# TopHillRobotics/quadruped-robot

Measured on AMD Instinct MI355X. Metric: MPC+WBC control ticks/s (batched robots), higher is better.
Workload: dtype f32 assembly / f64 QP+WBC

## Files before the change

### quadruped-robot_amd/csrc/qr_wbc_kernel.hip

```cpp
#include <hip/hip_runtime.h>
#include <type_traits>
#include "qr_device_types.h"
#include "qr_wave_helpers.h"
#include "qr_kernels.h"
#include "qr_wbc_rigid_body.h"

namespace qrgpu {

#ifdef QR_TIMELINE
#define QW_P_TL pipe.tl
#define QW_P_TLR pipe.tlr
#else
#define QW_P_TL ((long long *)nullptr)
#define QW_P_TLR ((int *)nullptr)
#endif

__device__ __forceinline__ real wsum(real v) { return wave_sum_d(v); }

__device__ __forceinline__ real dot18(const real *a, int as, const real *b, int bs, int k)
{
    real av[18], bv[18];
#pragma unroll
    for (int t = 0; t < 18; ++t) { const bool ok = t < k; av[t] = ok ? a[t * as] : 0.0; bv[t] = ok ? b[t * bs] : 0.0; }
    real s0 = 0.0, s1 = 0.0, s2 = 0.0;
#pragma unroll
    for (int t = 0; t < 18; t += 3) { s0 += av[t] * bv[t]; s1 += av[t + 1] * bv[t + 1]; s2 += av[t + 2] * bv[t + 2]; }
    return (s0 + s1) + s2;
}

__device__ __forceinline__ int fdiv16(int e, int rcp) { return (e * rcp) >> 16; }
__device__ __forceinline__ int rcp16(int n) { return (65536 + n - 1) / n; }

template <int KMAX>
__device__ __forceinline__ void gemm(int lane, real *C, int ldc, const real *A, int lda, bool tA, const real *B, int ldb, bool tB,
                                     int m, int n, int k, real alpha = 1.0, real beta = 0.0, const real *C0 = nullptr, int ldc0 = 0)
{
    const int rn = rcp16(n);
    const int as = tA ? lda : 1, bs = tB ? 1 : ldb;
    for (int e = lane; e < m * n; e += 64) {
        const int i = fdiv16(e, rn), j = e - i * n;
        const real *ap = tA ? A + i : A + i * lda;
        const real *bp = tB ? B + j * ldb : B + j;
        real av[KMAX], bv[KMAX];
#pragma unroll
        for (int t = 0; t < KMAX; ++t) { const bool ok = t < k; av[t] = ok ? ap[t * as] : 0.0; bv[t] = ok ? bp[t * bs] : 0.0; }
        real a0 = 0.0, a1 = 0.0, a2 = 0.0;
#pragma unroll
        for (int t = 0; t < KMAX; t += 3) {
            a0 += av[t] * bv[t];
            if (t + 1 < KMAX) a1 += av[t + 1] * bv[t + 1];
            if (t + 2 < KMAX) a2 += av[t + 2] * bv[t + 2];
        }
        real v = alpha * ((a0 + a1) + a2);
        if (C0) v += beta * C0[i * ldc0 + j];
        C[i * ldc + j] = v;
    }
    wave_sync();
}

template <int UMAX>
__device__ __forceinline__ real spd_inverse(int lane, real *A, int ld, int n, real *col)
{
    const int rn = rcp16(n);
    int ei[UMAX], ej[UMAX];
    real a[UMAX];
#pragma unroll
    for (int u = 0; u < UMAX; ++u) {
        const int e = lane + 64 * u;
        const bool ok = e < n * n;
        ei[u] = ok ? fdiv16(e, rn) : -1;
        ej[u] = ok ? e - ei[u] * n : -1;
        a[u] = ok ? A[ei[u] * ld + ej[u]] : 0.0;
    }
    real minpiv = 1e300;
    for (int k = 0; k < n; ++k) {
#pragma unroll
        for (int u = 0; u < UMAX; ++u) if (ej[u] == k) col[ei[u]] = a[u];
        wave_sync();
        const real piv = col[k];
        minpiv = piv < minpiv ? piv : minpiv;
        const real ip = fast_rcp(piv);
        real ci[UMAX], cj[UMAX];
#pragma unroll
        for (int u = 0; u < UMAX; ++u) { const bool ok = ei[u] >= 0; ci[u] = ok ? col[ei[u]] : 0.0; cj[u] = ok ? col[ej[u]] : 0.0; }
#pragma unroll
        for (int u = 0; u < UMAX; ++u) {
            if (ei[u] == k) a[u] = (ej[u] == k) ? -ip : cj[u] * ip;
            else if (ej[u] == k) a[u] = ci[u] * ip;
            else a[u] -= ci[u] * cj[u] * ip;
        }
        wave_sync();
    }
#pragma unroll
    for (int u = 0; u < UMAX; ++u) if (ei[u] >= 0) A[ei[u] * ld + ej[u]] = -a[u];
    wave_sync();
    return minpiv;
}

template <int UMAX = 3>
__device__ __forceinline__ void psd_pinv(int lane, const real *W, int n, real thr, real *Winv, real *scr)
{
    if (n == 1) {
        if (lane == 0) Winv[0] = (W[0] > thr) ? 1.0 / W[0] : 0.0;
        wave_sync();
        return;
    }
    for (int e = lane; e < n * n; e += 64) Winv[e] = W[e];
    wave_sync();
    const real minpiv = spd_inverse<UMAX>(lane, Winv, n, n, scr);
    real fro = 0.0;
    for (int e = lane; e < n * n; e += 64) fro += Winv[e] * Winv[e];
    fro = wsum(fro);
    const bool full_rank = (minpiv > 0.0) && (fro == fro) && (1.0 > thr * __builtin_sqrt(fro));
    if (full_rank) return;
    if (lane == 0) {
        real *Am = scr;
        real *V = Winv;
        for (int i = 0; i < n; ++i)
            for (int j = 0; j < n; ++j) { Am[i * n + j] = 0.5 * (W[i * n + j] + W[j * n + i]); V[i * n + j] = (i == j) ? 1.0 : 0.0; }
        for (int sweep = 0; sweep < 30; ++sweep) {
            real off = 0.0;
            for (int p = 0; p < n; ++p) for (int q2 = p + 1; q2 < n; ++q2) off += Am[p * n + q2] * Am[p * n + q2];
            if (off < 1e-40) break;
            for (int p = 0; p < n - 1; ++p)
                for (int q2 = p + 1; q2 < n; ++q2) {
                    const real apq = Am[p * n + q2];
                    if (apq == 0.0) continue;
                    const real th = (Am[q2 * n + q2] - Am[p * n + p]) / (2.0 * apq);
                    const real t = (th >= 0 ? 1.0 : -1.0) / (fabs(th) + __builtin_sqrt(th * th + 1.0));
                    const real c = 1.0 / __builtin_sqrt(t * t + 1.0), s = t * c;
                    for (int k = 0; k < n; ++k) { const real akp = Am[k * n + p], akq = Am[k * n + q2]; Am[k * n + p] = c * akp - s * akq; Am[k * n + q2] = s * akp + c * akq; }
                    for (int k = 0; k < n; ++k) { const real apk = Am[p * n + k], aqk = Am[q2 * n + k]; Am[p * n + k] = c * apk - s * aqk; Am[q2 * n + k] = s * apk + c * aqk; }
                    for (int k = 0; k < n; ++k) { const real vkp = V[k * n + p], vkq = V[k * n + q2]; V[k * n + p] = c * vkp - s * vkq; V[k * n + q2] = s * vkp + c * vkq; }
                }
        }
        real *ev = scr + n * n;
        for (int i = 0; i < n; ++i) { const real l = fabs(Am[i * n + i]); ev[i] = (l > thr) ? 1.0 / Am[i * n + i] : 0.0; }
        for (int i = 0; i < n; ++i) for (int j = 0; j < n; ++j) Am[i * n + j] = V[i * n + j] * ev[j];
        real *tmp = scr + n * n + n;
        for (int i = 0; i < n; ++i) for (int j = 0; j < n; ++j) { real a = 0; for (int k = 0; k < n; ++k) a += Am[i * n + k] * V[j * n + k]; tmp[i * n + j] = a; }
        for (int e = 0; e < n * n; ++e) Winv[e] = tmp[e];
    }
    wave_sync();
}

__device__ __forceinline__ bool sym3_inverse(const real *W, real thr, real iv[6])
{
    const real a = W[0], b = W[3], c = W[4], d = W[6], e = W[7], f = W[8];
    const real c00 = c * f - e * e, c10 = d * e - b * f, c20 = b * e - c * d, c11 = a * f - d * d, c21 = b * d - a * e, c22 = a * c - b * b;
    const real det = a * c00 + b * c10 + d * c20;
    const real id = 1.0 / det;
    iv[0] = c00 * id; iv[1] = c10 * id; iv[2] = c11 * id; iv[3] = c20 * id; iv[4] = c21 * id; iv[5] = c22 * id;
    const real fro = (iv[0] * iv[0] + iv[2] * iv[2] + iv[5] * iv[5]) + 2.0 * (iv[1] * iv[1] + iv[3] * iv[3] + iv[4] * iv[4]);
    return (a > 0.0) && (c22 > 0.0) && (det > 0.0) && (fro == fro) && (1.0 > thr * __builtin_sqrt(fro));
}

#define QW_NP    0
#define QW_T1    324
#define QW_JB    540
#define QW_JTP   756
#define QW_JTB   810
#define QW_T2    864
#define QW_LAM   918
#define QW_LAMI  1062
#define QW_SCR   1206
#define QW_VEC   1510
#define QW_QP    1564
#define QW_SIZE  1746
#define QR_WBC_SHARED_DOUBLES 1392
#define QR_WBC_LDS_DOUBLES (QR_WBC_SHARED_DOUBLES + 2 * QW_SIZE)

struct QpWork {
    real *tv;
    real *Nq;
    real *Sq;
    real *qd_, *qr_, *qu_, *qc0;
    real *qx;
};
__device__ __forceinline__ QpWork qp_work(real *W)
{
    QpWork q;
    q.tv = W + QW_VEC + 18; q.Nq = W + QW_NP; q.Sq = W + QW_JB;
    q.qd_ = W + QW_QP; q.qr_ = q.qd_ + 32; q.qu_ = q.qr_ + 32; q.qc0 = q.qu_ + 32; q.qx = q.qc0 + 32;
    return q;
}

#define CLEG(k) ((int)((cpack >> (4 * (k))) & 15u))
#define TLEG(k) ((int)((tpack >> (4 * (k))) & 15u))

__device__ __forceinline__ void wbc_signal_done(int *finished, int lane)
{
    if (!finished) return;
    asm volatile("s_waitcnt vmcnt(0)" ::: "memory");
    if (lane == 0) __hip_atomic_fetch_add(finished, 1, __ATOMIC_RELAXED, __HIP_MEMORY_SCOPE_AGENT);
}

__device__ __forceinline__ bool wbc_qp_setup(const int lane, const WbcConst &K, const int nc, const real *A, const real *JC, const real *qdd, const real *Cv, const real *Gv,
                                             real *W, int *sI)
{
    const int dimFr = 3 * nc;
    const QpWork Q = qp_work(W);
    real *tv = Q.tv, *Nq = Q.Nq, *Sq = Q.Sq, *qd_ = Q.qd_, *qx = Q.qx;
    const int nz = 6 + dimFr, np_ = 6, mi = 6 * nc;
    if (lane < 18) {
        real acc = Cv[lane] + Gv[lane];
        for (int k = 0; k < 18; ++k) acc += A[lane * 18 + k] * qdd[k];
        tv[lane] = acc;
    }
    for (int e = lane; e < (np_ + mi) * nz; e += 64) {
        const int c = e / nz, j = e - c * nz;
        real v = 0.0;
        if (c < 6) v = (j < 6) ? A[c * 18 + j] : -JC[(j - 6) * 18 + c];
        else {
            const int u = c - 6, k = u / 6, tt = u - 6 * k;
            if (j >= 6 && (j - 6) / 3 == k) {
                const int ax = (j - 6) - 3 * k;
                if (tt == 0) v = (ax == 2) ? 1.0 : 0.0;
                else if (tt == 5) v = (ax == 2) ? -1.0 : 0.0;
                else { const int a2 = (tt - 1) >> 1; v = (ax == a2) ? (((tt - 1) & 1) ? -1.0 : 1.0) : ((ax == 2) ? (real)K.mu : 0.0); }
            }
        }
        Nq[c * 18 + j] = v;
    }
    if (lane < 18) qx[lane] = 0.0;
    if (lane < 32) sI[32 + lane] = -1;
    wave_sync();
    const real iw_fb = 1.0 / (real)K.w_fb, iw_fr = 1.0 / (real)K.w_fr;
    if (lane < 36) {
        const int a = lane / 6, b2 = lane - 6 * a;
        real acc = 0.0;
        for (int j = 0; j < nz; ++j) acc += Nq[a * 18 + j] * ((j < 6) ? iw_fb : iw_fr) * Nq[b2 * 18 + j];
        Sq[a * 18 + b2] = acc;
    }
    wave_sync();
    real tr = 0.0;
#pragma unroll
    for (int a = 0; a < 6; ++a) tr += Sq[a * 18 + a];
    const real minpiv = spd_inverse<1>(lane, Sq, 18, 6, qd_);
    return !(minpiv > 1e-14 * tr);
}

__device__ __forceinline__ void wbc_qp_and_store(const int lane, const int rid, const int n, const WbcConst &K, const int nc, const unsigned cpack, const bool bad_type,
                                                 const bool eq_dependent, const real *A, const real *JC, const real *cm, real *W, int *sI,
                                                 float *__restrict__ g_tau, int *__restrict__ g_status, const int merge_tau, const int status_or, const int epilogue,
                                                 long long *__restrict__ dbgT, float *__restrict__ g_qp, const bool piped = false, float *__restrict__ g_prev = nullptr)
{
#define QW_TSF(i) do { if (dbgT && (threadIdx.x & 63) == 0 && threadIdx.x < 64) dbgT[(size_t)blockIdx.x * 16 + (i)] = clock64(); } while (0)
    int qp_iters = 0;
    const int dimFr = 3 * nc;
    const QpWork Q = qp_work(W);
    real *tv = Q.tv, *Nq = Q.Nq, *Sq = Q.Sq, *qd_ = Q.qd_, *qr_ = Q.qr_, *qu_ = Q.qu_, *qc0 = Q.qc0, *qx = Q.qx;
    const int nz = 6 + dimFr, np_ = 6, mi = 6 * nc;
    if (lane < 18) {
        real acc = tv[lane];
        for (int k = 0; k < dimFr; ++k) acc -= JC[k * 18 + lane] * cm[51 + 3 * CLEG(k / 3) + k % 3];
        tv[lane] = acc;
    }
    wave_sync();
    if (lane < np_ + mi) {
        const int c = lane;
        real v;
        if (c < 6) v = tv[c];
        else {
            const int u = c - 6, k = u / 6, tt = u - 6 * k;
            real acc = 0.0;
            for (int ax = 0; ax < 3; ++ax) acc += Nq[c * 18 + 6 + 3 * k + ax] * cm[51 + 3 * CLEG(k) + ax];
            v = acc - ((tt == 5) ? -(real)K.max_fz : 0.0);
        }
        qc0[c] = v;
    }
    wave_sync();
    int stw = bad_type ? QRGPU_ST_BAD_TYPE : 0;
    {
        int q = 0;
        const real iw_fb = 1.0 / (real)K.w_fb, iw_fr = 1.0 / (real)K.w_fr;
        auto Minv = [&](int j) -> real { return (j < 6) ? iw_fb : iw_fr; };
        int iter = 0;
        const int maxit = 200;
        int *iter_out = &qp_iters;
        bool fail = false;
        int *act = sI;
        int *posi = sI + 32;
        int next_eq = 0;
        {
            if (eq_dependent) { stw |= QRGPU_ST_WBC_INFEAS; fail = true; }
            if (lane < 6) {
                real acc = 0.0;
#pragma unroll
                for (int b2 = 0; b2 < 6; ++b2) acc -= Sq[lane * 18 + b2] * qc0[b2];
                qu_[lane] = acc; act[lane] = lane; posi[lane] = lane;
            }
            wave_sync();
            if (lane < nz) {
                real acc = 0.0;
#pragma unroll
                for (int a = 0; a < 6; ++a) acc += Nq[a * 18 + lane] * qu_[a];
                qx[lane] = Minv(lane) * acc;
            }
            q = 6; next_eq = np_;
            wave_sync();
        }
        int act_r = (lane < 6) ? lane : 0;
        real u_r = (lane < 6) ? qu_[lane] : 0.0;
        bool active_c = lane < 6;
        const real INF_ = __builtin_inf();
        while (!fail) {
            int p;
            {
                real bs = -1e-10; bool cand = false;
                if (lane >= 6 && lane < np_ + mi && !active_c) {
                    const int cj = 6 + 3 * ((lane - 6) / 6);
                    const real s_ = qc0[lane] + (Nq[lane * 18 + cj] * qx[cj] + Nq[lane * 18 + cj + 1] * qx[cj + 1] + Nq[lane * 18 + cj + 2] * qx[cj + 2]);
                    if (s_ < bs) { bs = s_; cand = true; }
                }
                const real mn = wave_min_d(bs);
                if (!(mn < -1e-10)) break;
                p = first_lane(cand && bs == mn);
                if (p < 0) break;
            }
            real up = 0.0;
            for (;;) {
                if (++iter > maxit) { stw |= QRGPU_ST_WBC_MAXITER; fail = true; break; }
                *iter_out = iter;
                const int pj = 6 + 3 * ((p - 6) / 6);
                const real pn0 = Nq[p * 18 + pj], pn1 = Nq[p * 18 + pj + 1], pn2 = Nq[p * 18 + pj + 2];
                const real delta = (pn0 * pn0 + pn1 * pn1 + pn2 * pn2) * iw_fr;
                const real w0 = iw_fr * pn0, w1 = iw_fr * pn1, w2 = iw_fr * pn2;
                real dq_ = 0.0;
                if (lane < q) { const real *na = Nq + act_r * 18 + pj; dq_ = na[0] * w0 + na[1] * w1 + na[2] * w2; }
                real rq_ = 0.0;
                {
                    const real *Srow = Sq + ((lane < q) ? lane : 0) * 18;
#pragma unroll
                    for (int c = 0; c < 18; c += 6) {
                        if (c >= q) continue;
                        real sv[6];
#pragma unroll
                        for (int j = 0; j < 6; ++j) sv[j] = Srow[c + j];
#pragma unroll
                        for (int j = 0; j < 6; ++j) rq_ += (c + j < q) ? sv[j] * readlane_d(dq_, c + j) : 0.0;
                    }
                    if (lane >= q) rq_ = 0.0;
                }
                const real dr = wave_sum_d(rq_ * dq_);
                const real zc = delta - dr;
                real t1; int lpos;
                {
                    const real tt = (lane < q && act_r >= np_ && rq_ > 0.0) ? u_r * fast_rcp(rq_) : INF_;
                    t1 = wave_min_d(tt);
                    lpos = (t1 < INF_) ? first_lane(tt == t1) : 0x7fffffff;
                }
                const real sp = qc0[p] + (pn0 * qx[pj] + pn1 * qx[pj + 1] + pn2 * qx[pj + 2]);
                const bool have_z = zc > 1e-13 * delta;
                const real izc = fast_rcp(zc);
                const real t2 = have_z ? -sp * izc : INF_;
                const real t = t1 < t2 ? t1 : t2;
                if (!(t < INF_)) { stw |= QRGPU_ST_WBC_INFEAS; fail = true; break; }
                if (have_z) {
                    real acc = 0.0;
                    const int lz = (lane < nz) ? lane : 0;
#pragma unroll
                    for (int c = 0; c < 18; c += 6) {
                        if (c >= q) continue;
                        real nv[6];
#pragma unroll
                        for (int j = 0; j < 6; ++j) nv[j] = Nq[__builtin_amdgcn_readlane(act_r, c + j) * 18 + lz];
#pragma unroll
                        for (int j = 0; j < 6; ++j) acc += (c + j < q) ? nv[j] * readlane_d(rq_, c + j) : 0.0;
                    }
                    if (lane < nz) {
                        const real wl_ = (lane == pj) ? w0 : (lane == pj + 1) ? w1 : (lane == pj + 2) ? w2 : 0.0;
                        qx[lane] += t * (wl_ - Minv(lane) * acc);
                    }
                }
                u_r -= t * rq_;
                up += t;
                if (have_z && t == t2) {
                    const real isg = izc;
                    if (lane < q) qr_[lane] = rq_;
                    wave_sync();
                    { const int rq2 = rcp16(q); for (int e = lane; e < q * q; e += 64) { const int i = fdiv16(e, rq2), j = e - i * q; Sq[i * 18 + j] += qr_[i] * qr_[j] * isg; } }
                    if (lane < q) { Sq[q * 18 + lane] = -rq_ * isg; Sq[lane * 18 + q] = -rq_ * isg; }
                    if (lane == 0) Sq[q * 18 + q] = isg;
                    if (lane == q) { act_r = p; u_r = up; }
                    if (lane == p) active_c = true;
                    ++q;
                    wave_sync();
                    break;
                }
                {
                    const int l = lpos, last = q - 1;
                    const int cdrop = __builtin_amdgcn_readlane(act_r, l), alast = __builtin_amdgcn_readlane(act_r, last);
                    const real ulast = readlane_d(u_r, last);
                    if (lane < q) qd_[lane] = Sq[lane * 18 + l];
                    wave_sync();
                    const real isl = 1.0 / qd_[l];
                    { const int rq2 = rcp16(q); for (int e = lane; e < q * q; e += 64) { const int i = fdiv16(e, rq2), j = e - i * q; if (i != l && j != l) Sq[i * 18 + j] -= qd_[i] * qd_[j] * isl; } }
                    wave_sync();
                    if (l != last) {
                        if (lane < last) qr_[lane] = (lane == l) ? Sq[last * 18 + last] : Sq[last * 18 + lane];
                        wave_sync();
                        if (lane < last) { Sq[l * 18 + lane] = qr_[lane]; Sq[lane * 18 + l] = qr_[lane]; }
                        if (lane == l) { act_r = alast; u_r = ulast; }
                    }
                    if (lane == cdrop) active_c = false;
                    --q;
                    wave_sync();
                }
            }
        }
    }

    QW_TSF(8);
    if (dbgT && threadIdx.x == 0) dbgT[(size_t)blockIdx.x * 16 + 10] = qp_iters;
    if (g_qp) {
        float *o = g_qp + (size_t)rid * 30;
        if (lane < 18) o[lane] = (lane < nz) ? (float)qx[lane] : 0.f;
        if (lane < 12) o[18 + lane] = (lane < dimFr) ? (float)(qx[6 + lane] + cm[51 + 3 * CLEG(lane / 3) + lane % 3]) : 0.f;
    }
    if (lane < 12) {
        const int row = 6 + lane;
        real acc = tv[row];
        for (int k = 0; k < 6; ++k) acc += A[row * 18 + k] * qx[k];
        for (int k = 0; k < dimFr; ++k) acc -= JC[k * 18 + row] * qx[6 + k];
        const int leg = lane / 3;
        const bool stance = cm[63 + leg] != 0.0;
        if (!epilogue) {
            if (!merge_tau || stance) st_through(&g_tau[(size_t)lane * n + rid], (float)acc, piped);
        } else {
            const float t = stance ? (float)acc
                                   : (piped ? __hip_atomic_load(g_tau + (size_t)lane * n + rid, __ATOMIC_RELAXED, __HIP_MEMORY_SCOPE_AGENT) : g_tau[(size_t)lane * n + rid]);
            st_through(&g_tau[(size_t)lane * n + rid], torque_epilogue(t, lane, !stance, epilogue), piped);
        }
    }
    if (g_prev && lane < 3) st_through(&g_prev[(size_t)lane * n + rid], (float)cm[12 + lane], piped);
    if (lane == 0 && g_status) {
        if (status_or & 2) stw |= QRGPU_ST_PIPE_TIMEOUT;
        if (status_or & 1) st_through(&g_status[rid], stw | (piped ? __hip_atomic_load(g_status + rid, __ATOMIC_RELAXED, __HIP_MEMORY_SCOPE_AGENT) : g_status[rid]), piped);
        else st_through(&g_status[rid], stw, piped);
    }
    QW_TSF(9);
#undef QW_TSF
}

#ifdef QR_WBC_DBG_BUILD
#define qr_wbc_kernel qr_wbc_kernel_dbg
#endif
__global__ __launch_bounds__(128, 2)
void qr_wbc_kernel(int n, const WbcConst *__restrict__ types, const int *__restrict__ type_id,
                   const float *__restrict__ g_state, const float *__restrict__ g_cmd, float *__restrict__ g_prev,
                   float *__restrict__ g_tau, float *__restrict__ g_qdes, int *__restrict__ g_status,
                   float *__restrict__ g_dbg, int merge_tau, int status_or, long long *__restrict__ dbgT,
                   const float *__restrict__ g_fr ,
                   int type_ready , int epilogue ,
                   float *__restrict__ g_qp ,
                   WbcPipe pipe )
{
#ifndef QR_WBC_DBG_BUILD
    dbgT = nullptr; g_dbg = nullptr; g_qp = nullptr;
#endif
#define QW_TS(i) do { if (dbgT && threadIdx.x == 0) dbgT[(size_t)blockIdx.x * 16 + (i)] = clock64(); } while (0)
#define QW_TS1(i) do { if (dbgT && threadIdx.x == 64) dbgT[(size_t)blockIdx.x * 16 + (i)] = clock64(); } while (0)
    QW_TS(0);
    int qp_iters = 0;
    int rid = xcd_robot_index((int)blockIdx.x + pipe.slot_base, n);
    const int lane = threadIdx.x & 63;
    const int wv = __builtin_amdgcn_readfirstlane((int)threadIdx.x >> 6);
    const bool gate_gave_up = pipe.gate_abort && __builtin_amdgcn_readfirstlane(*pipe.gate_abort) == (int)pipe.epoch;
    if (pipe.second) {
        if (!gate_gave_up) {
            int cnt = pipe.list_count ? *pipe.list_count : 0;
            cnt = cnt < n ? cnt : n;
            if ((int)blockIdx.x >= cnt) return;
            rid = pipe.list[blockIdx.x];
        }
    }
    if (rid < 0) return;
    if (!pipe.second && gate_gave_up) { wbc_signal_done(pipe.finished, lane); return; }
    if (QW_P_TL && threadIdx.x == 0 && !pipe.second) atomicMin(QW_P_TL + QR_TL_TICKS + (pipe.epoch & 63u) * 8 + 3, wall_clock64());
    if (pipe.order && !pipe.second) rid = pipe.order[rid];
    if (QW_P_TLR && threadIdx.x == 0 && !pipe.second) QW_P_TLR[rid] = (int)wall_clock64();
    int tyid = type_id ? type_id[rid] : 0;
    const bool bad_type = resolve_type(tyid, type_ready);
    const WbcConst &K = types[tyid & (QRGPU_MAX_TYPES - 1)];

    __shared__ real sm[QR_WBC_LDS_DOUBLES];
    real *A = sm;
    real *Ai = A + 324;
    real *JcA = Ai + 324;
    real *JC = JcA + 216;
    real *st = JC + 216;
    real *cm = st + 40;
    real *Gv = cm + 68;
    real *Cv = Gv + 18;
    real *Jcd = Cv + 18;
    real *pGC = Jcd + 12;
    real *vGC = pGC + 12;
    real *tkX = vGC + 12;
    real *tkE = tkX + 18;
    real *tkV = tkE + 18;
    real *legB = tkV + 18;
    real *sRT = legB + 64;
    real *W = sm + QR_WBC_SHARED_DOUBLES + wv * QW_SIZE;
    real *Np = W + QW_NP, *T1 = W + QW_T1, *JB = W + QW_JB, *JtP = W + QW_JTP, *JtB = W + QW_JTB, *T2 = W + QW_T2;
    real *lam = W + QW_LAM, *lamI = W + QW_LAMI, *scr = W + QW_SCR;
    real *qdd = W + QW_VEC, *tv = qdd + 18;
    real *dq1 = qdd, *dq2 = tv;
    __shared__ int sI[64];
    __shared__ int sPipe;
    if (threadIdx.x == 0) sPipe = 0;

    if (wv == 0) {
        if (lane < 37) st[lane] = (real)g_state[(size_t)lane * n + rid];
        for (int e = lane; e < 324; e += 64) A[e] = 0.0;
        for (int e = lane; e < 216; e += 64) JcA[e] = 0.0;
    } else if (g_tau) {
        for (int i = lane; i < 67; i += 64) cm[i] = (real)((g_fr && i >= 51 && i < 63) ? (pipe.flag ? 0.f : g_fr[(size_t)(i - 51) * n + rid]) : g_cmd[(size_t)i * n + rid]);
    }
    __syncthreads();
    const real *quat = st, *pos = st + 4, *bv = st + 7, *qj = st + 13, *qdj = st + 25;
    const xform3 Rwb = quat_to_rot_wb(quat);
    int nc = 0, nt = 2;
    unsigned cpack = 0, tpack = 0;
    if (g_tau) {
#pragma unroll
        for (int l = 0; l < 4; ++l) {
            const int in_contact = __builtin_amdgcn_readfirstlane(cm[63 + l] != 0.0 ? 1 : 0);
            if (in_contact) { cpack |= (unsigned)l << (4 * nc); ++nc; } else { tpack |= (unsigned)l << (4 * (nt - 2)); ++nt; }
        }
    }
    const int dimFr = 3 * nc;

    {
        real *sS = scr + 160, *sC = scr + 176;
        if (lane < 15) {
            const real th = (lane < 12) ? qj[lane] : ((wv == 1 && g_tau) ? cm[9 + lane - 12] : 0.0);
            real s_, c_;
            sincos(th, &s_, &c_);
            sS[lane] = s_; sC[lane] = c_;
        }
        wave_sync();
    }
    const real *sS = scr + 160, *sC = scr + 176;

    QW_TS(1);
    if (wv == 0) {
      if (lane < 4) wbc_leg_inertia_chain(K, Rwb, sS, sC, lane, A, JcA, Gv, legB);
      wave_sync();
      QW_TS(2);
      if (lane == 0) wbc_base_block(K, Rwb, legB, A, Gv);
      wave_sync();
      QW_TS(3);
    } else {
      if (lane < 4) wbc_leg_velocity_chain(K, Rwb, pos, bv, qdj, sS, sC, lane, pGC, vGC, Jcd, Cv, legB);
      wave_sync();
    }
    if (wv == 0) {
    {
        real *Tm = scr, *Um = scr + 72;
        if (lane < 36) {
            const int l = lane / 9, e = lane - 9 * l, i = e / 3, j = e - 3 * i;
            const real *B = A + (6 + 3 * l) * 18 + 6 + 3 * l;
            const real b00 = B[0], b01 = B[1], b02 = B[2], b11 = B[19], b12 = B[20], b22 = B[38];
            const real c00 = b11 * b22 - b12 * b12, c01 = b02 * b12 - b01 * b22, c02 = b01 * b12 - b02 * b11;
            const real c11 = b00 * b22 - b02 * b02, c12 = b01 * b02 - b00 * b12, c22 = b00 * b11 - b01 * b01;
            const real idet = 1.0 / (b00 * c00 + b01 * c01 + b02 * c02);
            const int lo = i < j ? i : j, hi = i < j ? j : i;
            const real c = (lo == 0) ? (hi == 0 ? c00 : (hi == 1 ? c01 : c02)) : (lo == 1 ? (hi == 1 ? c11 : c12) : c22);
            Um[lane] = c * idet;
        }
        wave_sync();
        for (int e = lane; e < 72; e += 64) {
            const int a = e / 12, c = e - 12 * a, l = c / 3, cc = c - 3 * l;
            const real *Ar = A + a * 18 + 6 + 3 * l, *Li = Um + 9 * l;
            Tm[e] = Ar[0] * Li[cc] + Ar[1] * Li[3 + cc] + Ar[2] * Li[6 + cc];
        }
        wave_sync();
        for (int e = lane; e < 144; e += 64) {
            const int c = e / 12, d = e - 12 * c;
            Ai[(6 + c) * 18 + 6 + d] = (c / 3 == d / 3) ? Um[9 * (c / 3) + 3 * (c % 3) + d % 3] : 0.0;
        }
        if (lane < 36) {
            const int a = lane / 6, b2 = lane - 6 * a;
            real acc = A[a * 18 + b2];
#pragma unroll
            for (int c = 0; c < 12; ++c) acc -= Tm[a * 12 + c] * A[b2 * 18 + 6 + c];
            Ai[a * 18 + b2] = acc;
        }
        wave_sync();
        spd_inverse<1>(lane, Ai, 18, 6, tv);
        for (int e = lane; e < 72; e += 64) {
            const int a = e / 12, c = e - 12 * a;
            real acc = 0.0;
#pragma unroll
            for (int b2 = 0; b2 < 6; ++b2) acc += Ai[a * 18 + b2] * Tm[b2 * 12 + c];
            Um[e] = acc;
            Ai[a * 18 + 6 + c] = -acc; Ai[(6 + c) * 18 + a] = -acc;
        }
        wave_sync();
        for (int e = lane; e < 144; e += 64) {
            const int c = e / 12, d = e - 12 * c;
            real acc = Ai[(6 + c) * 18 + 6 + d];
#pragma unroll
            for (int a = 0; a < 6; ++a) acc += Tm[a * 12 + c] * Um[a * 12 + d];
            Ai[(6 + c) * 18 + 6 + d] = acc;
        }
        wave_sync();
    }

      QW_TS(4);
      for (int e = lane; e < 54 * nc; e += 64) { const int k = e / 54; JC[e] = JcA[54 * CLEG(k) + (e - 54 * k)]; }
#pragma unroll
      for (int e = 0; e < 9; ++e) if (lane == e) sRT[e] = Rwb.m[e % 3][e / 3];
    } else {
      if (lane == 0) wbc_base_coriolis(K, bv, legB, Cv);
      if (lane == 0 && g_tau) {
        const xform3 RotT = transpose(Rwb);
        {
            const xform3 Rr = mul(mul(coord_rot_sc(0, sS[12], sC[12]), coord_rot_sc(1, sS[13], sC[13])), coord_rot_sc(2, sS[14], sC[14]));
            const xform3 r = transpose(Rr);
            real qd4[4];
            const real tr = r.m[0][0] + r.m[1][1] + r.m[2][2];
            if (tr > 0.0) {
                const real S = __builtin_sqrt(tr + 1.0) * 2.0;
                qd4[0] = 0.25 * S; qd4[1] = (r.m[2][1] - r.m[1][2]) / S; qd4[2] = (r.m[0][2] - r.m[2][0]) / S; qd4[3] = (r.m[1][0] - r.m[0][1]) / S;
            } else if ((r.m[0][0] > r.m[1][1]) && (r.m[0][0] > r.m[2][2])) {
                const real S = __builtin_sqrt(1.0 + r.m[0][0] - r.m[1][1] - r.m[2][2]) * 2.0;
                qd4[0] = (r.m[2][1] - r.m[1][2]) / S; qd4[1] = 0.25 * S; qd4[2] = (r.m[0][1] + r.m[1][0]) / S; qd4[3] = (r.m[0][2] + r.m[2][0]) / S;
            } else if (r.m[1][1] > r.m[2][2]) {
                const real S = __builtin_sqrt(1.0 + r.m[1][1] - r.m[0][0] - r.m[2][2]) * 2.0;
                qd4[0] = (r.m[0][2] - r.m[2][0]) / S; qd4[1] = (r.m[0][1] + r.m[1][0]) / S; qd4[2] = 0.25 * S; qd4[3] = (r.m[1][2] + r.m[2][1]) / S;
            } else {
                const real S = __builtin_sqrt(1.0 + r.m[2][2] - r.m[0][0] - r.m[1][1]) * 2.0;
                qd4[0] = (r.m[1][0] - r.m[0][1]) / S; qd4[1] = (r.m[0][2] + r.m[2][0]) / S; qd4[2] = (r.m[1][2] + r.m[2][1]) / S; qd4[3] = 0.25 * S;
            }
            const real r1 = qd4[0], r2 = quat[0];
            const v3 v1 = mk(qd4[1], qd4[2], qd4[3]), v2 = mk(-quat[1], -quat[2], -quat[3]);
            real e0 = r1 * r2 - dot(v1, v2);
            v3 ev = r1 * v2 + r2 * v1 + cross(v1, v2);
            if (e0 < 0.0) { e0 = -e0; ev = (-1.0) * ev; }
            v3 so3 = ev;
            const real theta = 2.0 * asin(__builtin_sqrt(dot(so3, so3)));
            if (fabs(theta) < 0.0000001) so3 = mk(0, 0, 0);
            else { const real sn = sin(theta / 2.0); so3 = (1.0 / sn) * so3; so3 = theta * so3; }
            if (pipe.wait_epoch) {
                const long long t0 = wall_clock64();
                int late = 0;
                for (;;) {
                    const unsigned w = __hip_atomic_load(pipe.wbc_done + rid, __ATOMIC_RELAXED, __HIP_MEMORY_SCOPE_AGENT);
                    if (qr_epoch_reached(w, pipe.wait_epoch)) break;
                    if (wall_clock64() - t0 > pipe.wait_ticks) { late = 1; break; }
                    __builtin_amdgcn_s_sleep(32);
                }
                if (lane == 0) sPipe = late;
            }
            auto prev_ld = [&](int i_) -> real {
                const float *p_ = g_prev + (size_t)i_ * n + rid;
                return (real)(pipe.wait_epoch ? __hip_atomic_load(p_, __ATOMIC_RELAXED, __HIP_MEMORY_SCOPE_AGENT) : *p_);
            };
            const v3 pv = mk(prev_ld(0), prev_ld(1), prev_ld(2));
            const v3 ve = mul(RotT, pv - mk(bv[0], bv[1], bv[2]));
            const real so[3] = {so3.x, so3.y, so3.z}, vev[3] = {ve.x, ve.y, ve.z};
#pragma unroll
            for (int i = 0; i < 3; ++i) {
                tkE[i] = so[i];
                tkV[i] = cm[12 + i];
                real x = K.kp_ori * so[i] + K.kd_ori * vev[i] + 0.0;
                tkX[i] = fmin(fmax(x, -10.0), 10.0);
            }
        }
        {
            const v3 vw = mul(RotT, mk(bv[3], bv[4], bv[5]));
            const real vwv[3] = {vw.x, vw.y, vw.z};
#pragma unroll
            for (int i = 0; i < 3; ++i) {
                const real pe = cm[i] - pos[i];
                tkE[3 + i] = pe;
                tkV[3 + i] = cm[3 + i];
                real x = K.kp_pos * pe + K.kd_pos * (cm[3 + i] - vwv[i]) + cm[6 + i];
                tkX[3 + i] = fmin(fmax(x, -10.0), 10.0);
            }
        }
        for (int t = 2; t < nt; ++t) {
            const int l = TLEG(t - 2);
            for (int i = 0; i < 3; ++i) {
                const real pe = cm[15 + 3 * l + i] - pGC[3 * l + i];
                tkE[3 * t + i] = pe;
                tkV[3 * t + i] = cm[27 + 3 * l + i];
                tkX[3 * t + i] = K.kp_foot * pe + K.kd_foot * (cm[27 + 3 * l + i] - vGC[3 * l + i]) + cm[39 + 3 * l + i];
            }
        }
    }
      QW_TS1(11);
    }
    __syncthreads();
    if (g_dbg) {
        if (wv == 0) {
            float *o = g_dbg + (size_t)rid * (324 + 18 + 18 + 216 + 36);
            for (int e = lane; e < 324; e += 64) o[e] = (float)A[e];
            if (lane < 18) { o[324 + lane] = (float)Gv[lane]; o[342 + lane] = (float)Cv[lane]; }
            for (int e = lane; e < 216; e += 64) o[360 + e] = (float)JcA[e];
            if (lane < 12) { o[576 + lane] = (float)Jcd[lane]; o[588 + lane] = (float)pGC[lane]; o[600 + lane] = (float)vGC[lane]; }
        }
        if (!g_tau) return;
    }
#define TASK_COLS(t, c0, J3, ld)                                                                           \
    const int c0 = ((t) == 0) ? 0 : ((t) == 1) ? 3 : 6 + 3 * TLEG((t) - 2);                                \
    const real *J3 = ((t) < 2) ? sRT : JcA + 54 * TLEG((t) - 2) + c0;                                      \
    const int ld = ((t) < 2) ? 3 : 18
    auto jt_npre = [&](const real *J3, int ld, int c0) {
        if (lane < 54) {
            const int i = lane / 18, j = lane - 18 * i;
            const real *nr = Np + c0 * 18 + j, *jr = J3 + i * ld;
            JtP[lane] = (jr[0] * nr[0] + jr[1] * nr[18]) + jr[2] * nr[36];
        }
        wave_sync();
    };
    auto npre_update = [&](const real *T) {
#pragma unroll
        for (int u = 0; u < 6; ++u) {
            const int e = lane + 64 * u;
            if (e < 324) {
                const int i = fdiv16(e, rcp16(18)), j = e - 18 * i;
                Np[e] -= (T[3 * i] * JtP[j] + T[3 * i + 1] * JtP[18 + j]) + T[3 * i + 2] * JtP[36 + j];
            }
        }
        wave_sync();
    };
    auto pinv3 = [&](real thr, real iv[6]) {
        if (!sym3_inverse(lam, thr, iv)) {
            psd_pinv(lane, lam, 3, thr, lamI, scr);
            iv[0] = lamI[0]; iv[1] = lamI[3]; iv[2] = lamI[4]; iv[3] = lamI[6]; iv[4] = lamI[7]; iv[5] = lamI[8];
        }
    };

    auto contact_part = [&](auto Dc, const bool dynamic, const real thr) {
        constexpr int D = decltype(Dc)::value;
        constexpr int UM = (D * D + 63) / 64;
        if (dynamic) {
            for (int e = lane; e < 18 * D; e += 64) { const int i = e / D, j = e - D * i; T1[e] = dot18(Ai + i * 18, 1, JC + j * 18, 1, 18); }
            wave_sync();
        }
        for (int e = lane; e < D * D; e += 64) {
            const int i = e / D, j = e - D * i;
            lam[e] = dynamic ? dot18(JC + i * 18, 1, T1 + j, D, 18) : dot18(JC + i * 18, 1, JC + j * 18, 1, 18);
        }
        wave_sync();
        psd_pinv<UM>(lane, lam, D, thr, lamI, scr);
        for (int e = lane; e < 18 * D; e += 64) {
            const int i = e / D, j = e - D * i;
            real av[D], bv[D];
#pragma unroll
            for (int k = 0; k < D; ++k) { av[k] = dynamic ? T1[i * D + k] : JC[k * 18 + i]; bv[k] = lamI[k * D + j]; }
            real a0 = 0.0, a1 = 0.0, a2 = 0.0;
#pragma unroll
            for (int k = 0; k < D; k += 3) { a0 += av[k] * bv[k]; a1 += av[k + 1] * bv[k + 1]; a2 += av[k + 2] * bv[k + 2]; }
            JB[e] = (a0 + a1) + a2;
        }
        wave_sync();
        if (dynamic && lane < 18) {
            real acc = 0.0;
#pragma unroll
            for (int k = 0; k < D; ++k) acc -= JB[lane * D + k] * Jcd[3 * CLEG(k / 3) + k % 3];
            qdd[lane] = acc;
        }
#pragma unroll
        for (int u = 0; u < 6; ++u) {
            const int e = lane + 64 * u;
            if (e < 324) {
                const int i = fdiv16(e, rcp16(18)), j = e - 18 * i;
                real av[D], bv[D];
#pragma unroll
                for (int k = 0; k < D; ++k) { av[k] = JB[i * D + k]; bv[k] = JC[k * 18 + j]; }
                real a0 = 0.0, a1 = 0.0, a2 = 0.0;
#pragma unroll
                for (int k = 0; k < D; k += 3) { a0 += av[k] * bv[k]; a1 += av[k + 1] * bv[k + 1]; a2 += av[k + 2] * bv[k + 2]; }
                Np[e] = ((i == j) ? 1.0 : 0.0) - ((a0 + a1) + a2);
            }
        }
        wave_sync();
    };

    QW_TS(5);
    if (wv == 1) {
      if (g_qdes) {
        const real thr2 = 1e-6;
        switch (nc) {
            case 1: contact_part(std::integral_constant<int, 3>{}, false, thr2); break;
            case 2: contact_part(std::integral_constant<int, 6>{}, false, thr2); break;
            case 3: contact_part(std::integral_constant<int, 9>{}, false, thr2); break;
            case 4: contact_part(std::integral_constant<int, 12>{}, false, thr2); break;
            default:
                for (int e = lane; e < 324; e += 64) Np[e] = ((e / 18) == (e % 18)) ? 1.0 : 0.0;
                wave_sync();
        }
        for (int t = 0; t < nt; ++t) {
            TASK_COLS(t, c0, J3, ld);
            jt_npre(J3, ld, c0);
            if (lane < 9) { const int a = lane / 3, b2 = lane - 3 * a; lam[lane] = dot18(JtP + a * 18, 1, JtP + b2 * 18, 1, 18); }
            wave_sync();
            real iv[6];
            pinv3(thr2, iv);
            if (lane < 54) {
                const int r = lane / 3, j = lane - 3 * r;
                const real i0 = j == 0 ? iv[0] : j == 1 ? iv[1] : iv[3], i1 = j == 0 ? iv[1] : j == 1 ? iv[2] : iv[4], i2 = j == 0 ? iv[3] : j == 1 ? iv[4] : iv[5];
                JtB[lane] = (JtP[r] * i0 + JtP[18 + r] * i1) + JtP[36 + r] * i2;
            }
            wave_sync();
            real upd = 0.0;
            if (lane < 36) {
                const int which = lane / 18, i = lane - 18 * which;
                const real *prevv = which ? dq2 : dq1;
                const real *tgt = which ? (tkV + 3 * t) : (tkE + 3 * t);
                real tv3[3];
#pragma unroll
                for (int k = 0; k < 3; ++k) {
                    tv3[k] = tgt[k];
                    if (t > 0) tv3[k] -= (J3[k * ld] * prevv[c0] + J3[k * ld + 1] * prevv[c0 + 1]) + J3[k * ld + 2] * prevv[c0 + 2];
                }
                upd = ((t > 0) ? prevv[i] : 0.0) + ((JtB[3 * i] * tv3[0] + JtB[3 * i + 1] * tv3[1]) + JtB[3 * i + 2] * tv3[2]);
            }
            if (t < nt - 1 && lane < 54) { const int r = lane / 3, j = lane - 3 * r; T1[lane] = dot18(Np + r * 18, 1, JtB + j, 3, 18); }
            wave_sync();
            if (lane < 36) { if (lane < 18) dq1[lane] = upd; else dq2[lane - 18] = upd; }
            if (t < nt - 1) npre_update(T1); else wave_sync();
        }
        if (lane < 12) {
            st_through(&g_qdes[(size_t)lane * n + rid], (float)(qj[lane] + dq1[6 + lane]), pipe.flag != nullptr);
            st_through(&g_qdes[(size_t)(12 + lane) * n + rid], (float)dq2[6 + lane], pipe.flag != nullptr);
        }
      }
      QW_TS1(13);
      wbc_signal_done(pipe.finished, lane);
      return;
    }

    const real thrW = 1e-4;
    switch (nc) {
        case 1: contact_part(std::integral_constant<int, 3>{}, true, thrW); break;
        case 2: contact_part(std::integral_constant<int, 6>{}, true, thrW); break;
        case 3: contact_part(std::integral_constant<int, 9>{}, true, thrW); break;
        case 4: contact_part(std::integral_constant<int, 12>{}, true, thrW); break;
        default:
            if (lane < 18) qdd[lane] = 0.0;
            for (int e = lane; e < 324; e += 64) Np[e] = ((e / 18) == (e % 18)) ? 1.0 : 0.0;
            wave_sync();
    }
    QW_TS(12);
    for (int t = 0; t < nt; ++t) {
        if (t == 1) QW_TS(14);
        TASK_COLS(t, c0, J3, ld);
        jt_npre(J3, ld, c0);
        if (lane < 54) { const int r = lane / 3, i = lane - 3 * r; T1[lane] = dot18(Ai + r * 18, 1, JtP + i * 18, 1, 18); }
        wave_sync();
        if (lane < 9) { const int a = lane / 3, b2 = lane - 3 * a; lam[lane] = dot18(JtP + a * 18, 1, T1 + b2, 3, 18); }
        wave_sync();
        real iv[6];
        pinv3(thrW, iv);
        if (lane < 54) {
            const int r = lane / 3, j = lane - 3 * r;
            const real i0 = j == 0 ? iv[0] : j == 1 ? iv[1] : iv[3], i1 = j == 0 ? iv[1] : j == 1 ? iv[2] : iv[4], i2 = j == 0 ? iv[3] : j == 1 ? iv[4] : iv[5];
            JtB[lane] = (T1[3 * r] * i0 + T1[3 * r + 1] * i1) + T1[3 * r + 2] * i2;
        }
        wave_sync();
        real upd = 0.0;
        if (lane < 18) {
            real tv3[3];
#pragma unroll
            for (int k = 0; k < 3; ++k)
                tv3[k] = tkX[3 * t + k] - ((t >= 2) ? Jcd[c0 - 6 + k] : 0.0) - ((J3[k * ld] * qdd[c0] + J3[k * ld + 1] * qdd[c0 + 1]) + J3[k * ld + 2] * qdd[c0 + 2]);
            upd = qdd[lane] + ((JtB[3 * lane] * tv3[0] + JtB[3 * lane + 1] * tv3[1]) + JtB[3 * lane + 2] * tv3[2]);
        }
        if (t < nt - 1 && lane < 54) { const int r = lane / 3, j = lane - 3 * r; T2[lane] = dot18(Np + r * 18, 1, JtB + j, 3, 18); }
        wave_sync();
        if (lane < 18) qdd[lane] = upd;
        if (t < nt - 1) npre_update(T2); else wave_sync();
    }

    QW_TS(7);
    const bool eq_dependent = wbc_qp_setup(lane, K, nc, A, JC, qdd, Cv, Gv, W, sI);
    int pipe_st = 0;
    if (pipe.flag) {
        unsigned v = 0;
        const long long t0 = wall_clock64();
        const long long list_ticks = pipe.wait_ticks > pipe.flag_ticks ? pipe.wait_ticks : pipe.flag_ticks;
        for (;;) {
            v = __hip_atomic_load(pipe.flag + rid, __ATOMIC_RELAXED, __HIP_MEMORY_SCOPE_AGENT);
            if ((v >> 1) == pipe.epoch && !(pipe.wait_list && (v & 1u))) break;
            if (wall_clock64() - t0 > (((v >> 1) == pipe.epoch && pipe.wait_list) ? list_ticks : pipe.flag_ticks)) {
                pipe_st = QRGPU_ST_PIPE_TIMEOUT;
                if (lane == 0) __hip_atomic_store(const_cast<unsigned *>(pipe.flag) + rid, 0x80000000u | (pipe.epoch << 1), __ATOMIC_RELAXED, __HIP_MEMORY_SCOPE_AGENT);
                break;
            }
            __builtin_amdgcn_s_sleep(32);
        }
        v = __builtin_amdgcn_readfirstlane(v);
        if (QW_P_TLR && lane == 0) QW_P_TLR[n + rid] = (int)wall_clock64();
        if (!pipe_st && (v & 1u)) { wbc_signal_done(pipe.finished, lane); return; }
        if (lane < 12) cm[51 + lane] = (real)__hip_atomic_load(g_fr + (size_t)lane * n + rid, __ATOMIC_RELAXED, __HIP_MEMORY_SCOPE_AGENT);
        wave_sync();
    }
    if (pipe.wait_epoch && ((volatile int *)&sPipe)[0]) pipe_st = QRGPU_ST_PIPE_TIMEOUT;
    wbc_qp_and_store(lane, rid, n, K, nc, cpack, bad_type, eq_dependent, A, JC, cm, W, sI, g_tau, g_status, merge_tau, status_or | (pipe_st ? 2 : 0), epilogue, dbgT, g_qp,
                     pipe.flag != nullptr || pipe.wbc_done != nullptr, g_prev);
    if (pipe.wbc_done) {
        asm volatile("s_waitcnt vmcnt(0)" ::: "memory");
        if (lane == 0) qr_epoch_raise(pipe.wbc_done + rid, pipe.epoch);
    }
    wbc_signal_done(pipe.finished, lane);
    if (QW_P_TL && lane == 0) atomicMax(QW_P_TL + QR_TL_TICKS + (pipe.epoch & 63u) * 8 + (pipe.second ? 7 : 4), wall_clock64());
    if (QW_P_TLR && lane == 0 && !pipe.second) QW_P_TLR[2 * n + rid] = (int)wall_clock64();
}

}
```

Baseline: 4.521 million.

## Restrict null-space projector updates to live task rows and register-stage WBC dot products

The null-space projector Np is now computed and updated only on the rows that later tasks still read (mapped through live_row), not on all 18x18 entries. The T1/T2 products are likewise limited to the remaining tasks. The QP setup builds the constraint matrix with a zero-fill pass followed by per-row writes, avoiding a per-element division and branching. Several dot products are staged into fixed-size register arrays and one active-set load is hoisted. The Jacobi fallback loops are kept un-unrolled to limit code size. The row-mapping logic is intricate and risks leaving stale projector rows if the live-row set is wrong.

```diff
diff --git a/quadruped-robot_amd/csrc/qr_wbc_kernel.hip b/quadruped-robot_amd/csrc/qr_wbc_kernel.hip
--- a/quadruped-robot_amd/csrc/qr_wbc_kernel.hip
+++ b/quadruped-robot_amd/csrc/qr_wbc_kernel.hip
@@ -135,10 +135,21 @@
                 }
         }
         real *ev = scr + n * n;
+#pragma unroll 1
         for (int i = 0; i < n; ++i) { const real l = fabs(Am[i * n + i]); ev[i] = (l > thr) ? 1.0 / Am[i * n + i] : 0.0; }
-        for (int i = 0; i < n; ++i) for (int j = 0; j < n; ++j) Am[i * n + j] = V[i * n + j] * ev[j];
+#pragma unroll 1
+        for (int e = 0; e < n * n; ++e) { const int j = e % n; Am[e] = V[e] * ev[j]; }
         real *tmp = scr + n * n + n;
-        for (int i = 0; i < n; ++i) for (int j = 0; j < n; ++j) { real a = 0; for (int k = 0; k < n; ++k) a += Am[i * n + k] * V[j * n + k]; tmp[i * n + j] = a; }
+#pragma unroll 1
+        for (int i = 0; i < n; ++i)
+#pragma unroll 1
+            for (int j = 0; j < n; ++j) {
+                real a = 0;
+#pragma unroll 1
+                for (int k = 0; k < n; ++k) a += Am[i * n + k] * V[j * n + k];
+                tmp[i * n + j] = a;
+            }
+#pragma unroll 1
         for (int e = 0; e < n * n; ++e) Winv[e] = tmp[e];
     }
     wave_sync();
@@ -203,24 +214,30 @@
     real *tv = Q.tv, *Nq = Q.Nq, *Sq = Q.Sq, *qd_ = Q.qd_, *qx = Q.qx;
     const int nz = 6 + dimFr, np_ = 6, mi = 6 * nc;
     if (lane < 18) {
+        real av[18], qv[18];
+#pragma unroll
+        for (int k = 0; k < 18; ++k) { av[k] = A[lane * 18 + k]; qv[k] = qdd[k]; }
         real acc = Cv[lane] + Gv[lane];
-        for (int k = 0; k < 18; ++k) acc += A[lane * 18 + k] * qdd[k];
+#pragma unroll
+        for (int k = 0; k < 18; ++k) acc += av[k] * qv[k];
         tv[lane] = acc;
     }
-    for (int e = lane; e < (np_ + mi) * nz; e += 64) {
-        const int c = e / nz, j = e - c * nz;
-        real v = 0.0;
-        if (c < 6) v = (j < 6) ? A[c * 18 + j] : -JC[(j - 6) * 18 + c];
-        else {
-            const int u = c - 6, k = u / 6, tt = u - 6 * k;
-            if (j >= 6 && (j - 6) / 3 == k) {
-                const int ax = (j - 6) - 3 * k;
-                if (tt == 0) v = (ax == 2) ? 1.0 : 0.0;
-                else if (tt == 5) v = (ax == 2) ? -1.0 : 0.0;
-                else { const int a2 = (tt - 1) >> 1; v = (ax == a2) ? (((tt - 1) & 1) ? -1.0 : 1.0) : ((ax == 2) ? (real)K.mu : 0.0); }
-            }
-        }
-        Nq[c * 18 + j] = v;
+#pragma unroll
+    for (int u = 0; u < 2; ++u) {
+        const int e = lane + 64 * u, c = e / 18, j = e - 18 * c;
+        if (e < 108 && j < nz) Nq[e] = (j < 6) ? A[c * 18 + j] : -JC[(j - 6) * 18 + c];
+    }
+    for (int e = lane; e < 9 * mi; e += 64) { Nq[108 + 2 * e] = 0.0; Nq[108 + 2 * e + 1] = 0.0; }
+    wave_sync();
+    if (lane < mi) {
+        const int k = lane / 6, tt = lane - 6 * k;
+        const int a2 = (tt - 1) >> 1;
+        const real sg = ((tt - 1) & 1) ? -1.0 : 1.0, ends = (tt == 0) ? 1.0 : -1.0;
+        const bool side = tt != 0 && tt != 5;
+        real *r = Nq + (6 + lane) * 18 + 6 + 3 * k;
+        r[0] = (side && a2 == 0) ? sg : 0.0;
+        r[1] = (side && a2 == 1) ? sg : 0.0;
+        r[2] = side ? (real)K.mu : ends;
     }
     if (lane < 18) qx[lane] = 0.0;
     if (lane < 32) sI[32 + lane] = -1;
@@ -228,8 +245,12 @@
     const real iw_fb = 1.0 / (real)K.w_fb, iw_fr = 1.0 / (real)K.w_fr;
     if (lane < 36) {
         const int a = lane / 6, b2 = lane - 6 * a;
+        real av[18], bv[18];
+#pragma unroll
+        for (int j = 0; j < 18; ++j) { const bool ok = j < nz; av[j] = ok ? Nq[a * 18 + j] : 0.0; bv[j] = ok ? Nq[b2 * 18 + j] : 0.0; }
         real acc = 0.0;
-        for (int j = 0; j < nz; ++j) acc += Nq[a * 18 + j] * ((j < 6) ? iw_fb : iw_fr) * Nq[b2 * 18 + j];
+#pragma unroll
+        for (int j = 0; j < 18; ++j) acc += av[j] * ((j < 6) ? iw_fb : iw_fr) * bv[j];
         Sq[a * 18 + b2] = acc;
     }
     wave_sync();
@@ -252,8 +273,12 @@
     real *tv = Q.tv, *Nq = Q.Nq, *Sq = Q.Sq, *qd_ = Q.qd_, *qr_ = Q.qr_, *qu_ = Q.qu_, *qc0 = Q.qc0, *qx = Q.qx;
     const int nz = 6 + dimFr, np_ = 6, mi = 6 * nc;
     if (lane < 18) {
+        real jv[12], fv[12];
+#pragma unroll
+        for (int k = 0; k < 12; ++k) { const bool ok = k < dimFr; jv[k] = ok ? JC[k * 18 + lane] : 0.0; fv[k] = ok ? cm[51 + 3 * CLEG(k / 3) + k % 3] : 0.0; }
         real acc = tv[lane];
-        for (int k = 0; k < dimFr; ++k) acc -= JC[k * 18 + lane] * cm[51 + 3 * CLEG(k / 3) + k % 3];
+#pragma unroll
+        for (int k = 0; k < 12; ++k) acc -= jv[k] * fv[k];
         tv[lane] = acc;
     }
     wave_sync();
@@ -324,19 +349,24 @@
                 *iter_out = iter;
                 const int pj = 6 + 3 * ((p - 6) / 6);
                 const real pn0 = Nq[p * 18 + pj], pn1 = Nq[p * 18 + pj + 1], pn2 = Nq[p * 18 + pj + 2];
+                const real qcp = qc0[p], qxp0 = qx[pj], qxp1 = qx[pj + 1], qxp2 = qx[pj + 2];
+                const real *Srow = Sq + ((lane < q) ? lane : 0) * 18;
+                const int lz = (lane < nz) ? lane : 0;
+                real sv0[6], nv0[6];
+#pragma unroll
+                for (int j = 0; j < 6; ++j) { sv0[j] = Srow[j]; nv0[j] = Nq[__builtin_amdgcn_readlane(act_r, j) * 18 + lz]; }
                 const real delta = (pn0 * pn0 + pn1 * pn1 + pn2 * pn2) * iw_fr;
                 const real w0 = iw_fr * pn0, w1 = iw_fr * pn1, w2 = iw_fr * pn2;
                 real dq_ = 0.0;
                 if (lane < q) { const real *na = Nq + act_r * 18 + pj; dq_ = na[0] * w0 + na[1] * w1 + na[2] * w2; }
                 real rq_ = 0.0;
                 {
-                    const real *Srow = Sq + ((lane < q) ? lane : 0) * 18;
 #pragma unroll
                     for (int c = 0; c < 18; c += 6) {
                         if (c >= q) continue;
                         real sv[6];
 #pragma unroll
-                        for (int j = 0; j < 6; ++j) sv[j] = Srow[c + j];
+                        for (int j = 0; j < 6; ++j) sv[j] = (c == 0) ? sv0[j] : Srow[c + j];
 #pragma unroll
                         for (int j = 0; j < 6; ++j) rq_ += (c + j < q) ? sv[j] * readlane_d(dq_, c + j) : 0.0;
                     }
@@ -350,7 +380,7 @@
                     t1 = wave_min_d(tt);
                     lpos = (t1 < INF_) ? first_lane(tt == t1) : 0x7fffffff;
                 }
-                const real sp = qc0[p] + (pn0 * qx[pj] + pn1 * qx[pj + 1] + pn2 * qx[pj + 2]);
+                const real sp = qcp + (pn0 * qxp0 + pn1 * qxp1 + pn2 * qxp2);
                 const bool have_z = zc > 1e-13 * delta;
                 const real izc = fast_rcp(zc);
                 const real t2 = have_z ? -sp * izc : INF_;
@@ -358,13 +388,12 @@
                 if (!(t < INF_)) { stw |= QRGPU_ST_WBC_INFEAS; fail = true; break; }
                 if (have_z) {
                     real acc = 0.0;
-                    const int lz = (lane < nz) ? lane : 0;
 #pragma unroll
                     for (int c = 0; c < 18; c += 6) {
                         if (c >= q) continue;
                         real nv[6];
 #pragma unroll
-                        for (int j = 0; j < 6; ++j) nv[j] = Nq[__builtin_amdgcn_readlane(act_r, c + j) * 18 + lz];
+                        for (int j = 0; j < 6; ++j) nv[j] = (c == 0) ? nv0[j] : Nq[__builtin_amdgcn_readlane(act_r, c + j) * 18 + lz];
 #pragma unroll
                         for (int j = 0; j < 6; ++j) acc += (c + j < q) ? nv[j] * readlane_d(rq_, c + j) : 0.0;
                     }
@@ -420,9 +449,16 @@
     }
     if (lane < 12) {
         const int row = 6 + lane;
+        real av[6], xv[6], jv[12], zv[12];
+#pragma unroll
+        for (int k = 0; k < 6; ++k) { av[k] = A[row * 18 + k]; xv[k] = qx[k]; }
+#pragma unroll
+        for (int k = 0; k < 12; ++k) { const bool ok = k < dimFr; jv[k] = ok ? JC[k * 18 + row] : 0.0; zv[k] = ok ? qx[6 + k] : 0.0; }
         real acc = tv[row];
-        for (int k = 0; k < 6; ++k) acc += A[row * 18 + k] * qx[k];
-        for (int k = 0; k < dimFr; ++k) acc -= JC[k * 18 + row] * qx[6 + k];
+#pragma unroll
+        for (int k = 0; k < 6; ++k) acc += av[k] * xv[k];
+#pragma unroll
+        for (int k = 0; k < 12; ++k) acc -= jv[k] * zv[k];
         const int leg = lane / 3;
         const bool stance = cm[63 + leg] != 0.0;
         if (!epilogue) {
@@ -716,15 +752,25 @@
         }
         wave_sync();
     };
-    auto npre_update = [&](const real *T) {
+    auto live_row = [&](int first, int m) -> int {
+        const int q3 = (m * 11) >> 5, tk = first + q3;
+        return ((tk == 0) ? 0 : (tk == 1) ? 3 : 6 + 3 * TLEG((tk - 2) & 3)) + (m - 3 * q3);
+    };
+    auto npre_update = [&](const real *T, int first) {
+        const int cnt = 54 * (nt - first);
 #pragma unroll
         for (int u = 0; u < 6; ++u) {
+            if (64 * u >= cnt) break;
             const int e = lane + 64 * u;
-            if (e < 324) {
-                const int i = fdiv16(e, rcp16(18)), j = e - 18 * i;
-                Np[e] -= (T[3 * i] * JtP[j] + T[3 * i + 1] * JtP[18 + j]) + T[3 * i + 2] * JtP[36 + j];
-            }
-        }
+            if (e < cnt) {
+                const int m = fdiv16(e, rcp16(18)), j = e - 18 * m, i = live_row(first, m);
+                Np[i * 18 + j] -= (T[3 * i] * JtP[j] + T[3 * i + 1] * JtP[18 + j]) + T[3 * i + 2] * JtP[36 + j];
+            }
+        }
+        wave_sync();
+    };
+    auto npre_identity = [&]() {
+        for (int e = lane; e < 54 * nt; e += 64) { const int m = fdiv16(e, rcp16(18)), j = e - 18 * m, i = live_row(0, m); Np[i * 18 + j] = (i == j) ? 1.0 : 0.0; }
         wave_sync();
     };
     auto pinv3 = [&](real thr, real iv[6]) {
@@ -764,18 +810,20 @@
             for (int k = 0; k < D; ++k) acc -= JB[lane * D + k] * Jcd[3 * CLEG(k / 3) + k % 3];
             qdd[lane] = acc;
         }
+        const int cnt = 54 * nt;
 #pragma unroll
         for (int u = 0; u < 6; ++u) {
+            if (64 * u >= cnt) break;
             const int e = lane + 64 * u;
-            if (e < 324) {
-                const int i = fdiv16(e, rcp16(18)), j = e - 18 * i;
+            if (e < cnt) {
+                const int m = fdiv16(e, rcp16(18)), j = e - 18 * m, i = live_row(0, m);
                 real av[D], bv[D];
 #pragma unroll
                 for (int k = 0; k < D; ++k) { av[k] = JB[i * D + k]; bv[k] = JC[k * 18 + j]; }
                 real a0 = 0.0, a1 = 0.0, a2 = 0.0;
 #pragma unroll
                 for (int k = 0; k < D; k += 3) { a0 += av[k] * bv[k]; a1 += av[k + 1] * bv[k + 1]; a2 += av[k + 2] * bv[k + 2]; }
-                Np[e] = ((i == j) ? 1.0 : 0.0) - ((a0 + a1) + a2);
+                Np[i * 18 + j] = ((i == j) ? 1.0 : 0.0) - ((a0 + a1) + a2);
             }
         }
         wave_sync();
@@ -790,9 +838,7 @@
             case 2: contact_part(std::integral_constant<int, 6>{}, false, thr2); break;
             case 3: contact_part(std::integral_constant<int, 9>{}, false, thr2); break;
             case 4: contact_part(std::integral_constant<int, 12>{}, false, thr2); break;
-            default:
-                for (int e = lane; e < 324; e += 64) Np[e] = ((e / 18) == (e % 18)) ? 1.0 : 0.0;
-                wave_sync();
+            default: npre_identity();
         }
         for (int t = 0; t < nt; ++t) {
             TASK_COLS(t, c0, J3, ld);
@@ -820,10 +866,10 @@
                 }
                 upd = ((t > 0) ? prevv[i] : 0.0) + ((JtB[3 * i] * tv3[0] + JtB[3 * i + 1] * tv3[1]) + JtB[3 * i + 2] * tv3[2]);
             }
-            if (t < nt - 1 && lane < 54) { const int r = lane / 3, j = lane - 3 * r; T1[lane] = dot18(Np + r * 18, 1, JtB + j, 3, 18); }
+            if (lane < 9 * (nt - 1 - t)) { const int m = lane / 3, j = lane - 3 * m, r = live_row(t + 1, m); T1[3 * r + j] = dot18(Np + r * 18, 1, JtB + j, 3, 18); }
             wave_sync();
             if (lane < 36) { if (lane < 18) dq1[lane] = upd; else dq2[lane - 18] = upd; }
-            if (t < nt - 1) npre_update(T1); else wave_sync();
+            if (t < nt - 1) npre_update(T1, t + 1); else wave_sync();
         }
         if (lane < 12) {
             st_through(&g_qdes[(size_t)lane * n + rid], (float)(qj[lane] + dq1[6 + lane]), pipe.flag != nullptr);
@@ -843,8 +889,7 @@
         case 4: contact_part(std::integral_constant<int, 12>{}, true, thrW); break;
         default:
             if (lane < 18) qdd[lane] = 0.0;
-            for (int e = lane; e < 324; e += 64) Np[e] = ((e / 18) == (e % 18)) ? 1.0 : 0.0;
-            wave_sync();
+            npre_identity();
     }
     QW_TS(12);
     for (int t = 0; t < nt; ++t) {
@@ -871,10 +916,10 @@
                 tv3[k] = tkX[3 * t + k] - ((t >= 2) ? Jcd[c0 - 6 + k] : 0.0) - ((J3[k * ld] * qdd[c0] + J3[k * ld + 1] * qdd[c0 + 1]) + J3[k * ld + 2] * qdd[c0 + 2]);
             upd = qdd[lane] + ((JtB[3 * lane] * tv3[0] + JtB[3 * lane + 1] * tv3[1]) + JtB[3 * lane + 2] * tv3[2]);
         }
-        if (t < nt - 1 && lane < 54) { const int r = lane / 3, j = lane - 3 * r; T2[lane] = dot18(Np + r * 18, 1, JtB + j, 3, 18); }
+        if (lane < 9 * (nt - 1 - t)) { const int m = lane / 3, j = lane - 3 * m, r = live_row(t + 1, m); T2[3 * r + j] = dot18(Np + r * 18, 1, JtB + j, 3, 18); }
         wave_sync();
         if (lane < 18) qdd[lane] = upd;
-        if (t < nt - 1) npre_update(T2); else wave_sync();
+        if (t < nt - 1) npre_update(T2, t + 1); else wave_sync();
     }
 
     QW_TS(7);
```

After: 4.583 million, median of 6. 1.01x the previous value.
